# Sreyan88/audio-ssl

Measured on AMD Instinct MI355X. Metric: upstream clips/sec (1s@16kHz, 64-mel), higher is better.
Workload: dtype bf16; 1 GPU; delores-m upstream step (log-mel + 2 views + q/k conv encoders + MoCo + 3 Barlow heads + bwd + SGD), 1 s @ 16 kHz, 64 mel, batch 512/GPU, queue 65536; global_batch=512, parallelism=dp1

## Files before the change

audio-ssl_amd/src/engine.py:

```python
import os

import torch

from src import _native as N

import os as _os
_STEM_VALU = _os.environ.get("AUDIOSSL_STEM_VALU") == "1"
BN_MOMENTUM = 0.1
BN_EPS = 1e-5
_BN_FUSED = _os.environ.get("AUDIOSSL_BN_FUSED", "1") != "0"


ONE_STREAM = os.environ.get("AUDIOSSL_ONE_STREAM", "0") == "1"


_CAPTURE_ORIGIN = []


class capture_scope:

    def __enter__(self):
        _CAPTURE_ORIGIN.append(torch.cuda.current_stream())
        return self

# ... 91 lines not shown
    n = src.numel()
    if src.dtype == torch.float32 and dst.dtype == torch.float32 and src.is_contiguous() and dst.is_contiguous() and n % 1024 == 0 \
            and n // 1024 < (1 << 31) and src.data_ptr() % 16 == 0 and dst.data_ptr() % 16 == 0:
        N.call("tile_rows", src, dst, n // 1024, n // 1024, 1, 1.0, 1024)
    else:
        dst.copy_(src)
    return dst


def _ksplit(M, Nn, K, target=512):
    tiles = ((M + 127) // 128) * ((Nn + 127) // 128)
    return int(max(1, min(target // max(tiles, 1), (K // 64) // 32)))


def gemm(dtype, ta, tb, M, Nn, K, A, lda, B, ldb, C, ldc, alpha=1.0, bias=None, relu=0, keep=None, ldk=0, keep_scale=1.0,
         gate=None, ldg=0, out_f32=0, atomic=0, ksplit=1, resid=None, ldr=0):
    N.call("gemm", dtype, ta, tb, M, Nn, K, float(alpha), A, lda, B, ldb, C, ldc, bias, relu, keep, ldk, float(keep_scale),
           gate, ldg, out_f32, atomic, ksplit, resid, ldr)


def linear_fwd(dtype, X, W, M, Nout, K, bias=None, relu=0, keep=None, keep_scale=1.0, out=None, out_f32=0):
    if out is None and dtype == N.BF16 and out_f32 and not relu and keep is None and M * Nout <= (1 << 16) and K >= 1024 and K % 512 == 0:
        out = ARENA.zeros((M, Nout), torch.float32, like=X)
        gemm(dtype, 0, 0, M, Nout, K, X, K, W, K, out, Nout, bias=bias, out_f32=1, atomic=1, ksplit=min(8, K // 256))
        return out
    if out is None:
        out = _empty((M, Nout), torch.float32 if (out_f32 or dtype == 0) else torch.bfloat16, like=X)
    gemm(dtype, 0, 0, M, Nout, K, X, K, W, K, out, Nout, bias=bias, relu=relu, keep=keep, ldk=Nout, keep_scale=keep_scale,
         out_f32=out_f32)
    return out


def linear_bwd_w(dtype, dY, X, dW, M, Nout, K, dw_zero=False):
    ks = _ksplit(Nout, K, M)
    atomic = 1 if (ks > 1 or dtype != N.BF16) else (0 if dw_zero else 2)
    gemm(dtype, 1, 1, Nout, K, M, dY, Nout, X, K, dW, K, out_f32=1, atomic=atomic, ksplit=ks)


def linear_bwd_x(dtype, dY, W, M, Nout, K, alpha=1.0, gate=None, out=None, out_f32=0):
    if out is None:
        out = _empty((M, K), torch.float32 if (out_f32 or dtype == N.F32) else torch.bfloat16, like=dY)
    gemm(dtype, 0, 1, M, K, Nout, dY, Nout, W, K, out, K, alpha=alpha, gate=gate, ldg=K, out_f32=out_f32)
    return out


GD = N.F32

HP = False


def set_high_precision(flag):
    global HP
    HP = bool(flag)


SYNC_BN = None


class SyncBN:
    def __init__(self, group=None):
        import torch.distributed as dist
        self.dist, self.group = dist, group
        self.world = dist.get_world_size(group)

    def all_reduce(self, t):
        self.dist.all_reduce(t, group=self.group)
        return t


def set_sync_bn(sync):
    global SYNC_BN
    SYNC_BN = sync if (sync is not None and sync.world > 1) else None


def _ad(dtype):
    return N.F32 if (HP or dtype == N.F32) else dtype


def pooled_dtype(dtype):
    return torch.float32


def center_cast(Y, groups, B):
    C = Y.shape[1]
    yc = _empty((groups * B, C), torch.bfloat16, like=Y)
    cmean = _empty((groups, C), torch.float32, like=Y)
    N.call("center_cast", Y, yc, cmean, groups, B, C)
    return yc, cmean


def colsum_add(dtype, X, M, C, dst, tmp=None):
    tmp = tmp if tmp is not None else ARENA.scratch((C,), torch.float64, X)
    N.call("colstats", dtype, X, 1, M, C, C, 0, tmp, None)
    N.call("add_d2f", tmp, dst, C)


def cast(dtype, src, n=None):
    if dtype == N.F32:
        return src
    out = torch.empty(src.shape, dtype=torch.bfloat16, device=src.device)
    N.call("cast", dtype, src, out, src.numel())
    return out


class EncoderCtx:
    pass


def _bn_train(dtype, Y, M, C, gamma, beta, rm, rv, update_running, groups=1):
    sq = ARENA.scratch((2, groups * C), torch.float64, Y)
    N.call("colstats", dtype, Y, groups, M, C, C, 1, sq[0], sq[1])
    if SYNC_BN is not None:
        SYNC_BN.all_reduce(sq)
        M = M * SYNC_BN.world
    st = _empty((4, groups * C), torch.float32, like=Y)
    N.call("bn_finalize", sq[0], sq[1], groups, float(M), C, gamma, beta, rm if update_running else None,
           rv if update_running else None, BN_MOMENTUM, BN_EPS, st[0], st[1], st[2], st[3])
    return st[0], st[1], st[2], st[3]


def bn_train_apply(dtype, ad, a, M, C, gamma, beta, rm, rv, update_running, groups, relu, out):
    if M <= 1024 and C % 32 == 0 and _BN_FUSED and SYNC_BN is None:
        st = _empty((4, groups * C), torch.float32, like=a)
        N.call("colbn_train_fwd", dtype, ad, a, gamma, beta, rm if update_running else None, rv if update_running else None,
               BN_MOMENTUM, BN_EPS, relu, groups, M, C, out, st[0], st[1], st[2], st[3])
        return st[0], st[1], st[2], st[3]
    st = _bn_train(ad, a, M, C, gamma, beta, rm, rv, update_running, groups)
    N.call("colbn_fwd", dtype, ad, a, st[0], st[1], relu, out, groups, M, C)
    return st


def _bn_eval(like, C, gamma, beta, rm, rv):
    scale, shift = _empty((C,), torch.float32, like=like), _empty((C,), torch.float32, like=like)
    N.call("bn_eval_affine", gamma, beta, rm, rv, BN_EPS, C, scale, shift)
    return scale, shift


_WGRAD_WS = {}


def _wgrad_workspace(device):
    key = device.index if device.index is not None else torch.cuda.current_device()
    ws = _WGRAD_WS.get(key)
    if ws is None:
        ws = _WGRAD_WS[key] = torch.empty(256 * 64 * 576, dtype=torch.float32, device=device)
    return ws


STAT_REPLICAS = 8
LOSS_REPLICAS = 32
_BN_STATS_P = os.environ.get("AUDIOSSL_BN_STATS_P", "1") != "0"
_DP1_BF16 = os.environ.get("AUDIOSSL_DP1_BF16", "1") != "0"
_CONV_POOL = os.environ.get("AUDIOSSL_CONV_POOL", "1") != "0"
_CONV_WS = int(os.environ.get("AUDIOSSL_CONV_WS", "1")) != 0


def _conv_block_fwd(dtype, Pin, Nimg, Ti, Fi, W, bias, bn, train, update_running, col, packed=None, keep_y=True):
    td = N.torch_dtype(dtype)
    if packed is not None:
        Wf, Wd = packed
    else:
        Wf, Wd = _empty((64, 576), td, like=Pin), _empty((64, 576), td, like=Pin)
        N.call("pack_conv_w", dtype, W, Wf, Wd)
    M = Nimg * Ti * Fi
    ad = _ad(dtype)
    gamma, beta, rm, rv = bn
    fused = dtype == N.BF16 and Fi in (16, 32)
    if fused and ad == dtype and _CONV_POOL and _CONV_WS and Ti % 2 == 0 and M * 128 < 0x7FFFFF00:
        rep = STAT_REPLICAS if (train and SYNC_BN is None) else 1
        sq = ARENA.scratch((rep, 2, 64), torch.float64, Pin)
        Y = _empty((M, 64), td, like=Pin) if keep_y else None
        Pout = _empty((Nimg, Ti // 2, Fi // 2, 64), td, like=Pin)
        N.call("conv3x3_pool_fwd", Pin, Wf, bias, gamma, Y, Pout, sq[0, 0], sq[0, 1], rep, Nimg, Ti, Fi)
        if train and SYNC_BN is None:
            st = _empty((4, 64), torch.float32, like=Pin)
            N.call("bn_relu_pooled_train_fwd", dtype, Pout, sq[0, 0], sq[0, 1], rep, float(M), gamma, beta, rm if update_running else None,
                   rv if update_running else None, BN_MOMENTUM, BN_EPS, Pout, st[0], st[1], st[2], st[3], Nimg, Ti // 2, Fi // 2)
            return Y, Pout, (st[0], st[1], st[2], st[3]), Wf, Wd
        if train:
            st = _empty((4, 64), torch.float32, like=Pin)
            sq = sq[0]
            SYNC_BN.all_reduce(sq)
            N.call("bn_finalize", sq[0], sq[1], 1, float(M * SYNC_BN.world), 64, gamma, beta, rm if update_running else None,
                   rv if update_running else None, BN_MOMENTUM, BN_EPS, st[0], st[1], st[2], st[3])
            scale, shift, mean, rstd = st[0], st[1], st[2], st[3]
        else:
            scale, shift = _bn_eval(Pin, 64, gamma, beta, rm, rv)
            mean = rstd = None
        N.call("bn_relu_pooled_fwd", dtype, Pout, scale, shift, Pout, Nimg, Ti // 2, Fi // 2)
        return Y, Pout, (scale, shift, mean, rstd), Wf, Wd
    Y = _empty((M, 64), N.torch_dtype(ad), like=Pin)
    rep = STAT_REPLICAS if (fused and train and SYNC_BN is None) else 1
    sq = ARENA.scratch((rep, 2, 64), torch.float64, Pin) if (fused and train) else None
    if fused:
        N.call("conv3x3_fwd", Pin, Wf, bias, Y, int(ad == N.F32), None if sq is None else sq[0, 0], None if sq is None else sq[0, 1],
               rep, Nimg, Ti, Fi)
    else:
        N.call("im2col3x3", dtype, Pin, col, Nimg, Ti, Fi)
        gemm(dtype, 0, 0, M, 64, 576, col, 576, Wf, 576, Y, 64, bias=bias, out_f32=int(ad == N.F32))
    Pout = _empty((Nimg, Ti // 2, Fi // 2, 64), td, like=Pin)
    if train and fused and SYNC_BN is None:
        st = _empty((4, 64), torch.float32, like=Pin)
        N.call("bn_relu_pool_train_fwd", dtype, ad, Y, sq[0, 0], sq[0, 1], rep, float(M), gamma, beta, rm if update_running else None,
               rv if update_running else None, BN_MOMENTUM, BN_EPS, Pout, st[0], st[1], st[2], st[3], Nimg, Ti, Fi)
        return Y, Pout, (st[0], st[1], st[2], st[3]), Wf, Wd
    if train and fused:
        st = _empty((4, 64), torch.float32, like=Pin)
        sq = sq[0]
        SYNC_BN.all_reduce(sq)
        N.call("bn_finalize", sq[0], sq[1], 1, float(M * SYNC_BN.world), 64, gamma, beta, rm if update_running else None,
               rv if update_running else None, BN_MOMENTUM, BN_EPS, st[0], st[1], st[2], st[3])
        scale, shift, mean, rstd = st[0], st[1], st[2], st[3]
    elif train:
        scale, shift, mean, rstd = _bn_train(ad, Y, M, 64, gamma, beta, rm, rv, update_running)
    else:
        scale, shift = _bn_eval(Y, 64, gamma, beta, rm, rv)
        mean = rstd = None
    N.call("bn_relu_pool_fwd", dtype, ad, Y, scale, shift, Pout, Nimg, Ti, Fi)
    return Y, Pout, (scale, shift, mean, rstd), Wf, Wd


def _col_buffer(dtype, Nimg, T1, F1, like):
    if dtype == N.BF16 and F1 in (16, 32):
        return None
    return _empty((Nimg * T1 * F1, 576), N.torch_dtype(dtype), like=like)


MOM_SLOT = 17 * 54


def stem_fused(dtype, train=True):
    return bool(train) and dtype == N.BF16 and not HP and not _STEM_VALU and SYNC_BN is None


def stem_moments_pair(xa, xb=None):
    Nimg, _, F, T = xa.shape
    assert xb is None or xb.shape == xa.shape
    mom = ARENA.scratch((1 if xb is None else 2, MOM_SLOT), torch.float64, xa)
    N.call("conv1_moments_pair", xa.reshape(Nimg, F, T).contiguous(), None if xb is None else xb.reshape(Nimg, F, T).contiguous(),
           Nimg, F, T, mom)
    return mom


def encoder_forward(P, x, dtype, keep=None, p_drop=0.3, train=True, update_running=True, want_layers=True, Wc=None,
                    layer_out=None, before_fc=None, stem_moments=None, need_bwd=True, lens=None, hop=160):
    Nimg, _, F, T = x.shape
    assert F == 64, "the HIP encoder is built for n_mels = 64 (the reference's only setting)"
    td = N.torch_dtype(dtype)
    c = EncoderCtx()
    c.P = P
    c.dtype, c.N, c.F, c.T, c.train, c.p_drop = dtype, Nimg, F, T, train, p_drop
    c.need_bwd = need_bwd
    ragged = lens is not None
    if ragged:
        assert not train and not need_bwd, "a ragged batch runs in eval mode without a backward (BatchNorm on running statistics)"
        assert T % 8 == 0, "a ragged batch is padded to a multiple of 8 frames"
        assert lens.dtype == torch.int32 and lens.is_cuda and tuple(lens.shape) == (Nimg,), "lens: int32 [N] on the device"
    img = x.reshape(Nimg, F, T).contiguous()
    c.img = img
    w1 = P["features_1.0.weight"].reshape(64, 9)
    b1 = P["features_1.0.bias"]
    g1, be1 = P["features_1.1.weight"], P["features_1.1.bias"]
    c.stem_mfma = dtype == N.BF16 and not HP and not _STEM_VALU
    fused = stem_fused(dtype, train)
    assert stem_moments is None or fused, "precomputed stem moments are for the fused bf16 training stem only"
    rm1 = rv1 = None
    if train:
        c.sc1, c.sh1, c.mean1, c.rstd1 = (_empty((64,), torch.float32, like=x) for _ in range(4))
        rm1 = P["features_1.1.running_mean"] if update_running else None
        rv1 = P["features_1.1.running_var"] if update_running else None
    if fused:
        c.mom1 = stem_moments if stem_moments is not None else stem_moments_pair(x)[0]
    elif train:
        c.mom1 = ARENA.scratch((16 * 54,), torch.float64, x)
        if SYNC_BN is None:
            N.call("conv1_stats", img, Nimg, F, T, w1, b1, g1, be1, rm1, rv1, BN_MOMENTUM, BN_EPS, c.mom1, c.sc1, c.sh1, c.mean1, c.rstd1)
        else:
            N.call("conv1_moments", img, Nimg, F, T, c.mom1)
            mom_g = SYNC_BN.all_reduce(c.mom1[:54].clone())
            N.call("conv1_finalize", mom_g, w1, b1, g1, be1, rm1, rv1, BN_MOMENTUM, BN_EPS, float(Nimg * F * T * SYNC_BN.world),
                   c.sc1, c.sh1, c.mean1, c.rstd1)
    else:
        c.sc1, c.sh1 = _bn_eval(x, 64, g1, be1, P["features_1.1.running_mean"], P["features_1.1.running_var"])
    T1, F1 = T // 2, F // 2
    c.P1 = _empty((Nimg, T1, F1, 64), td, like=x)
    x1 = x2 = x3 = None
    if want_layers:
        x1, x2, x3 = layer_out if layer_out is not None else (_empty((Nimg, f * 64), torch.float32 if ragged else td, like=x)
                                                              for f in (F // 2, F // 4, F // 8))
    x1_fused = c.stem_mfma and x1 is not None and x1.dtype == torch.float32 and x1.is_contiguous() and not ragged
    x1_parts = _empty((4, Nimg, (F // 2) * 64), torch.float32, like=x) if x1_fused else None
    if fused:
        N.call("conv1_fwd_train", img, Nimg, F, T, c.mom1, float(Nimg * F * T), w1, b1, g1, be1, rm1, rv1, BN_MOMENTUM, BN_EPS,
               c.sc1, c.sh1, c.mean1, c.rstd1, c.P1, x1_parts)
    else:
        N.call("conv1_fwd", dtype if (dtype == N.F32 or c.stem_mfma) else 2, img, Nimg, F, T, w1, b1, c.sc1, c.sh1, c.P1, x1_parts)
    if ragged:
        N.call("tail_mask", dtype, c.P1, lens, hop, 1, Nimg, T1, F1 * 64)
    col = _col_buffer(dtype, Nimg, T1, F1, x)
    bn2 = (P["features_2.1.weight"], P["features_2.1.bias"], P["features_2.1.running_mean"], P["features_2.1.running_var"])
    packs = [_empty((64, 576), td, like=x) for _ in range(4)]
    N.call("pack_conv_w2", dtype, P["features_2.0.weight"], packs[0], packs[1], P["features_3.0.weight"], packs[2], packs[3])
    c.Y2, c.P2, c.st2, c.W2f, c.W2d = _conv_block_fwd(dtype, c.P1, Nimg, T1, F1, P["features_2.0.weight"],
                                                       P["features_2.0.bias"], bn2, train, update_running, col, packed=packs[:2],
                                                       keep_y=need_bwd)
    T2, F2 = T1 // 2, F1 // 2
# ... 311 lines not shown
    vp = ctypes.c_void_p
    arrs = (_harr(ctypes.c_int, Ns), _harr(ctypes.c_int, Ks), _harr(vp, As), _harr(ctypes.c_long, ldas), _harr(vp, Bs),
            _harr(ctypes.c_long, ldbs), _harr(vp, Ps), _harr(vp, Moms), _harr(vp, Shadows if Shadows is not None else [None] * n),
            _harr(ctypes.c_long, ldps))
    if N.PROFILE is not None:
        N.PROFILE_NOTE = (float(sum(2.0 * M * nn * kk for nn, kk in zip(Ns, Ks))),
                          float(sum(2.0 * kk * (M + nn) + M * nn * (16.0 + (2.0 if Shadows is not None else 0.0)) for nn, kk in zip(Ns, Ks))))
    lr, mu, wd, gs, gs_dev = hyper
    N.call("gemm_multi_sgd", n, ta, tb, M, adr(arrs[0]), adr(arrs[1]), float(alpha), adr(arrs[2]), adr(arrs[3]), adr(arrs[4]), adr(arrs[5]),
           adr(arrs[6]), adr(arrs[7]), adr(arrs[8]), adr(arrs[9]), float(lr), float(mu), float(wd), float(gs), gs_dev)


def _heads_wgrad_split(D, kmax, M, nh):
    return _ksplit(D, kmax, M, max(256 // nh, 1))


def heads_wgrads_store(D, kins, M, grads_zero=True):
    nh = len(kins)
    return bool(grads_zero) and all(_heads_wgrad_split(D, k, M, nh) == 1 for k in (D, max(kins)))


def barlow_heads_forward_backward(PPs, Gs, Ys, dtype, lambds, scale_losses, loss_outs, update_running=True, backward=True,
                                  Wcs=None, grads_zero=False, dy_ready=None, sgd=None):
    import ctypes
    nh = len(Ys)
    B = Ys[0].shape[0] // 2
    M = 2 * B
    td = N.torch_dtype(dtype)
    dev = Ys[0].device
    W = Wcs if Wcs is not None else [tuple(cast(dtype, PP[f"projector.{i}.weight"]) for i in (0, 3, 6)) for PP in PPs]
    D = W[0][0].shape[0]
    kins = [Y.shape[1] for Y in Ys]
    ad = _ad(dtype)
    if dtype != N.BF16 or ad != N.BF16 or B > 1024 or D % 32:
        raise RuntimeError("grouped Barlow heads: bf16 path with B <= 1024 only")
    H = range(nh)
    vp, fl, adr = ctypes.c_void_p, ctypes.c_float, ctypes.addressof
    new = lambda rows, cols, t: [torch.empty(rows, cols, dtype=t, device=dev) for _ in H]

    def layer(xs, ws, ks, prefix, affine, relu):
        a = new(M, D, td)
        gemm_multi(0, 0, M, D, ks, xs, ks, ws, ks, a, D)
        out, st = new(M, D, td), new(4, 2 * D, torch.float32)
        par = lambda suffix, on=True: _harr(vp, [PP[prefix + suffix] if on else None for PP in PPs])
        arrs = (_harr(vp, a), par(".weight", affine), par(".bias", affine), par(".running_mean", update_running),
                par(".running_var", update_running), _harr(vp, out), _harr(vp, st))
        _multi_check(a, out, st)
        N.call("colbn_train_fwd_multi", nh, ad, adr(arrs[0]), adr(arrs[1]), adr(arrs[2]), adr(arrs[3]), adr(arrs[4]),
               BN_MOMENTUM, BN_EPS, relu, 2, B, D, adr(arrs[5]), adr(arrs[6]))
        return a, st, out
    ycs = [torch.empty(M, k, dtype=torch.bfloat16, device=dev) for k in kins]
    cms = [torch.empty(2, k, dtype=torch.float32, device=dev) for k in kins]
    _multi_check(list(Ys), ycs, cms)
    if any(Y.dtype != torch.float32 or k % 32 for Y, k in zip(Ys, kins)):
        raise RuntimeError("grouped Barlow heads: fp32 inputs with width % 32 == 0")
    arrs = (_harr(vp, list(Ys)), _harr(vp, ycs), _harr(vp, cms), _harr(ctypes.c_int, kins))
    N.call("center_cast_multi", nh, adr(arrs[0]), adr(arrs[1]), adr(arrs[2]), adr(arrs[3]), 2, B)
    a1, st1, h1 = layer(ycs, [W[h][0] for h in H], kins, "projector.1", True, 1)

    def shift_running():
        rms = [PP["projector.1.running_mean"] for PP in PPs]
        w0 = [W[h][0] for h in H]
        _multi_check(w0, rms)
        arrs = (_harr(vp, w0), _harr(vp, cms), _harr(vp, rms), _harr(ctypes.c_int, kins))
        N.call("shift_running_mean_multi", nh, adr(arrs[0]), adr(arrs[1]), adr(arrs[2]), D, adr(arrs[3]), 2, BN_MOMENTUM)
    shift_late = update_running and backward and dy_ready is not None
    if update_running and not shift_late:
        shift_running()
    a2, st2, h2 = layer(h1, [W[h][1] for h in H], [D] * nh, "projector.4", True, 1)
    z, st0, zn = layer(h2, [W[h][2] for h in H], [D] * nh, "bn", False, 0)
    dc = new(D, D, td)
    coefs = [(lambds[h] if lambds[h] else 1.0) * scale_losses[h] for h in H]
    dsc = [2.0 * c / B for c in coefs]
    if all(l.numel() == LOSS_REPLICAS for l in loss_outs) and D % 64 == 0:
        _multi_check([zn[h] for h in H], dc, list(loss_outs))
        arrs = (_harr(ctypes.c_int, [B] * nh), _harr(vp, [zn[h][:B] for h in H]), _harr(ctypes.c_long, [D] * nh),
                _harr(vp, [zn[h][B:] for h in H]), _harr(ctypes.c_long, [D] * nh), _harr(vp, dc), _harr(fl, coefs), _harr(fl, dsc),
                _harr(vp, list(loss_outs)))
        if N.PROFILE is not None:
            N.PROFILE_NOTE = float(nh * 2.0 * D * D * B)
        N.call("gemm_multi_barlow", nh, D, adr(arrs[0]), 1.0 / B, adr(arrs[1]), adr(arrs[2]), adr(arrs[3]), adr(arrs[4]), adr(arrs[5]),
               adr(arrs[6]), adr(arrs[7]), adr(arrs[8]))
    else:
        cm = new(D, D, torch.float32)
        gemm_multi(1, 1, D, D, [B] * nh, [zn[h][:B] for h in H], [D] * nh, [zn[h][B:] for h in H], [D] * nh, cm, D,
                   alpha=1.0 / B, out_f32=1)
        arrs = (_harr(vp, cm), _harr(fl, coefs), _harr(fl, dsc), _harr(vp, dc), _harr(vp, list(loss_outs)))
        _multi_check(list(loss_outs))
        N.call("barlow_loss_multi", nh, adr(arrs[0]), D, adr(arrs[1]), adr(arrs[2]), adr(arrs[3]), adr(arrs[4]))
    if not backward:
        return [None] * nh
    dzn = new(M, D, torch.float32)
    gemm_multi(0, 0, B, D, [D] * nh, [zn[h][B:] for h in H], [D] * nh, dc, [D] * nh, [dzn[h][:B] for h in H], D, out_f32=1)
    gemm_multi(0, 1, B, D, [D] * nh, [zn[h][:B] for h in H], [D] * nh, dc, [D] * nh, [dzn[h][B:] for h in H], D, out_f32=1)

    def bn_bwd(a, dh, st, relu, names):
        out = new(M, D, td)
        grads = lambda k: _harr(vp, [Gs[h][names[k]] if names else None for h in H])
        arrs = (_harr(vp, a), _harr(vp, dh), _harr(vp, st), _harr(vp, out), grads(0), grads(1))
        _multi_check(a, dh, st)
        N.call("colbn_bwd_multi", nh, ad, GD, adr(arrs[0]), adr(arrs[1]), adr(arrs[2]), relu, 2, B, D, adr(arrs[3]),
               adr(arrs[4]), adr(arrs[5]))
        return out

    def wgrad(dys, xs, name, ks):
        split = _heads_wgrad_split(D, max(ks), M, nh)
        if sgd is not None:
            if split != 1 or Wcs is None:
                raise RuntimeError("fused SGD needs unsplit weight gradients and the flat weight shadows")
            li = {"projector.0.weight": 0, "projector.3.weight": 1, "projector.6.weight": 2}[name]
            gemm_multi_sgd(1, 1, D, ks, [M] * nh, dys, [D] * nh, xs, ks, [PPs[h][name] for h in H], [sgd["momentum"][h][name] for h in H],
                           [W[h][li] for h in H], ks, sgd["hyper"])
            return
        gemm_multi(1, 1, D, ks, [M] * nh, dys, [D] * nh, xs, ks, [Gs[h][name] for h in H], ks, out_f32=1,
                   atomic=1 if split > 1 else (0 if grads_zero else 2), ksplit=split)

    def dgrad(dys, ws, Ks, rows):
        out = [torch.empty(rows, k, dtype=torch.float32, device=dev) for k in Ks]
        gemm_multi(0, 1, rows, Ks, [D] * nh, [dy[:rows] for dy in dys], [D] * nh, ws, Ks, out, Ks, out_f32=1)
        return out
    later = []
    defer = (lambda fn: later.append(fn)) if dy_ready is not None else (lambda fn: fn())
    dz = bn_bwd(z, dzn, st0, 0, None)
    defer(lambda: wgrad(dz, h2, "projector.6.weight", [D] * nh))
    dh2 = dgrad(dz, [W[h][2] for h in H], [D] * nh, M)
    da2 = bn_bwd(a2, dh2, st2, 1, ("projector.4.weight", "projector.4.bias"))
    defer(lambda: wgrad(da2, h1, "projector.3.weight", [D] * nh))
    dh1 = dgrad(da2, [W[h][1] for h in H], [D] * nh, M)
    da1 = bn_bwd(a1, dh1, st1, 1, ("projector.1.weight", "projector.1.bias"))
    defer(lambda: wgrad(da1, ycs, "projector.0.weight", kins))
    dy = dgrad(da1, [W[h][0] for h in H], kins, B)
    if dy_ready is not None:
        dy_ready()
    if shift_late:
        shift_running()
    for fn in later:
        fn()
    return dy


def moco_forward_backward(dtype, q, k, queue, queue_shadow, temperature, loss_out, backward=True):
    B, dim = q.shape
    K = queue.shape[1]
    td = N.torch_dtype(dtype)
    qn, kn = _empty((B, dim), td, like=q), _empty((B, dim), td, like=q)
    qn32, kn32 = _empty((B, dim), torch.float32, like=q), _empty((B, dim), torch.float32, like=q)
    qinv, kinv = _empty((B,), torch.float32, like=q), _empty((B,), torch.float32, like=q)
    lpos = _empty((B,), torch.float32, like=q)
    N.call("moco_prep", dtype, q, k, B, dim, 1.0 / temperature, qn, qn32, qinv, kn, kn32, kinv, lpos)
    lse = _empty((B,), torch.float32, like=q)
    dlpos = _empty((B,), torch.float32, like=q)
    Pm = None
    if dtype == N.BF16 and K % 8 == 0 and dim % 8 == 0:
        nslot = (K + 63) // 64
        part = _empty((B, nslot, 2), torch.float32, like=q)
        N.call("moco_logits", 1, qn, queue_shadow, B, K, dim, 1.0 / temperature, part, None, 0.0, None)
        N.call("moco_lse_merge", lpos, part, B, nslot, 1.0 / (B * temperature), lse, loss_out, dlpos)
        if not backward:
            return None, kn32
        Pm = _empty((B, K), td, like=q)
        N.call("moco_logits", 2, qn, queue_shadow, B, K, dim, 1.0 / temperature, None, lse, 1.0 / (B * temperature), Pm)
    else:
        lneg = _empty((B, K), torch.float32, like=q)
        gemm(dtype, 0, 1, B, K, dim, qn, dim, queue_shadow, K, lneg, K, alpha=1.0 / temperature, out_f32=1)
        N.call("moco_ce_fwd", lpos, lneg, B, K, lse, loss_out)
        if not backward:
            return None, kn32
        Pm = _empty((B, K), td, like=q)
        N.call("moco_ce_bwd", dtype, lpos, lneg, lse, B, K, 1.0 / (B * temperature), Pm, dlpos)
    dqn = ARENA.zeros((B, dim), torch.float32, device=q.device)
    gemm(dtype, 0, 0, B, dim, K, Pm, K, queue_shadow, K, dqn, dim, out_f32=1, atomic=1, ksplit=_ksplit(B, dim, K, 256))
    dq = _empty((B, dim), td, like=q)
    N.call("l2norm_bwd", dtype, dqn, dlpos, kn32, qn32, qinv, B, dim, dq)
    return dq, kn32
```

include/audiossl_hip.h:

```cpp
#ifndef AUDIOSSL_HIP_H
#define AUDIOSSL_HIP_H

#include <stdint.h>

#ifdef __cplusplus
extern "C" {
#endif

#define AUDIOSSL_OK 0
#define AUDIOSSL_EINVAL (-1)
#define AUDIOSSL_ELAUNCH (-2)
#define AUDIOSSL_EALIGN (-3)

int audiossl_logmel_fwd(const float* wave, float* out, int B, int L, int T, int n_fft, int hop, int n_mels, int taps,
                        const float* win, const float* tw, const float* melw, const int* mel_start, float eps_pow,
                        float eps_log, int apply_log, void* stream);
int audiossl_logmel_ragged_fwd(const float* wave, const int* lens, const int* lens_host, float* out, int B, int Lmax, int Tmax,
                               int n_fft, int hop, int n_mels, int taps, const float* win, const float* tw, const float* melw,
                               const int* mel_start, float eps_pow, float eps_log, int apply_log, void* stream);

int audiossl_fbank_fwd(const float* wave, const int* lens, const int* partner, const float* lam, float* clip_mean,
                       const int* bands, const int* bands_host, float* out, int B, int Lmax, int win_len, int shift, int n_fft, int n_mels,
                       int taps, int T_target, const float* win, const float* tw, const float* melw, const int* mel_start,
                       float preemph, float eps_log, float mean, float std, int skip_norm, int time_major, void* stream);
// ... 15 lines not shown
                           const int* off_r, const double* eta_l, const double* eta_r, const double* win, const double* delta,
                           int nwin, int index_step, void* stream);

int audiossl_pcm_window(const void* pcm, long pcm_bytes, const long long* tab, const long long* tab_host, float* out, int B,
                        int unit, int align, void* stream);

int audiossl_kmix_cluster(const float* views, const float* centroids, int n_views, int F, int T, int K, int* cluster,
                          void* stream);
int audiossl_kmix_apply(const float* views, const float* ring, const int* slot, const float* coef, int n_views, int n,
                        int log_mix, float* out, void* stream);
int audiossl_mask_fill(float* x, const int* tab, int n_img, int max_masks, int F, int T, int zero_fill, void* stream);

int audiossl_conv1_stats(const float* img, int N, int F, int T, const float* w, const float* bias, const float* gamma,
                         const float* beta, float* running_mean, float* running_var, float momentum, float eps,
                         double* mom, float* scale, float* shift, float* save_mean, float* save_rstd, void* stream);
#define AUDIOSSL_CONV1_XL_PARTS 4
int audiossl_conv1_fwd(int dtype, const float* img, int N, int F, int T, const float* w, const float* bias,
                       const float* scale, const float* shift, void* out, float* xl, void* stream);
#define AUDIOSSL_CONV1_MOM_SLOT (17 * 54)
int audiossl_conv1_moments_pair(const float* img_a, const float* img_b, int N, int F, int T, double* mom, void* stream);
int audiossl_conv1_fwd_train(const float* img, int N, int F, int T, double* mom, double count, const float* w, const float* bias,
                             const float* gamma, const float* beta, float* running_mean, float* running_var, float momentum,
                             float eps, float* scale, float* shift, float* save_mean, float* save_rstd, void* out, float* xl,
                             void* stream);
int audiossl_conv1_bwd(int dtype, int conv_dtype, const float* img, int N, int F, int T, const float* w, const float* bias,
                       const float* gamma, const float* scale, const float* shift, const float* mean, const float* rstd,
                       const double* mom, const void* dP, const void* dxl, float* acc, float* dW, float* dbias,
                       float* dgamma, float* dbeta, void* stream);

int audiossl_colstats(int dtype, const void* x, int groups, long M, int C, long ld, int want_sq, double* sum,
                      double* sumsq, void* stream);
int audiossl_bn_finalize(const double* sum, const double* sumsq, int groups, double count, int C, const float* gamma,
                         const float* beta, float* running_mean, float* running_var, float momentum, float eps,
                         float* scale, float* shift, float* save_mean, float* save_rstd, void* stream);
int audiossl_bn_relu_pool_fwd(int dtype, int ydtype, const void* Y, const float* scale, const float* shift, void* P, int N,
                              int Ti, int Fi, void* stream);
int audiossl_bn_relu_pool_train_fwd(int dtype, int ydtype, const void* Y, const double* sum, const double* sumsq, int stat_replicas,
                                    double count, const float* gamma, const float* beta, float* running_mean, float* running_var,
                                    float momentum, float eps, void* P, float* scale, float* shift, float* save_mean, float* save_rstd,
                                    int N, int Ti, int Fi, void* stream);
int audiossl_bn_relu_pooled_fwd(int dtype, const void* Praw, const float* scale, const float* shift, void* P, int N, int To, int Fo,
                                void* stream);
int audiossl_bn_relu_pooled_train_fwd(int dtype, const void* Praw, const double* sum, const double* sumsq, int stat_replicas,
                                      double count, const float* gamma, const float* beta, float* running_mean, float* running_var,
                                      float momentum, float eps, void* P, float* scale, float* shift, float* save_mean,
                                      float* save_rstd, int N, int To, int Fo, void* stream);
int audiossl_tmean_fwd(int dtype, int out_f32, const void* P, void* xl, int N, int To, int Fo, void* stream);
int audiossl_tmean3_fwd(int dtype, int out_f32, const void* P1, void* x1, const float* x1_parts, int To1, int Fo1, const void* P2,
                        void* x2, int To2, int Fo2, const void* P3, void* x3, int To3, int Fo3, int N, void* stream);
int audiossl_bn_relu_pool_bwd(int dtype, int ydtype, int gdtype, const void* Y, const void* dP, const void* dxl, const float* scale,
                              const float* shift, const float* mean, const float* rstd, float* stat, void* dY,
                              float* dgamma, float* dbeta, int N, int Ti, int Fi, void* stream);
int audiossl_bn_relu_pool_bwd_p(int dtype, int ydtype, int gdtype, const void* Y, const void* P, const void* dP, const void* dxl,
                                const float* scale, const float* shift, const float* mean, const float* rstd, float* stat, void* dY,
                                float* dgamma, float* dbeta, int N, int Ti, int Fi, void* stream);
int audiossl_conv1_moments(const float* img, int N, int F, int T, double* mom, void* stream);
int audiossl_conv1_finalize(double* mom_totals, const float* w, const float* bias, const float* gamma, const float* beta,
                            float* running_mean, float* running_var, float momentum, float eps, double count, float* scale,
                            float* shift, float* save_mean, float* save_rstd, void* stream);
int audiossl_conv1_bwd_sums(int dtype, int conv_dtype, const float* img, int N, int F, int T, const float* w, const float* bias,
                            const float* gamma, const float* scale, const float* shift, const float* mean, const float* rstd,
                            const double* mom, const void* dP, const void* dxl, float* acc, float* lstat, void* stream);
int audiossl_conv1_bwd_finalize(const float* acc, const double* mom, const float* w, const float* bias, const float* gamma,
                                const float* mean, const float* rstd, double count_global, const float* gstat, float* dW,
                                float* dbias, float* dgamma, float* dbeta, void* stream);
int audiossl_bn_relu_pool_bwd_stats(int dtype, int ydtype, int gdtype, const void* Y, const void* dP, const void* dxl,
                                    const float* scale, const float* shift, const float* mean, const float* rstd, float* stat,
                                    int N, int Ti, int Fi, void* stream);
int audiossl_bn_relu_pool_bwd_apply(int dtype, int ydtype, int gdtype, const void* Y, const void* dP, const void* dxl,
                                    const float* scale, const float* shift, const float* mean, const float* rstd, float* stat,
                                    const float* gstat, double count_global, void* dY, float* dgamma, float* dbeta, int N, int Ti,
                                    int Fi, void* stream);
int audiossl_colbn_bwd_stats(int dtype, int adtype, int gdtype, const void* a, const void* dh, const float* scale,
                             const float* shift, const float* mean, const float* rstd, int relu, int groups, long M, int C,
                             double* tmp, void* stream);
int audiossl_colbn_bwd_apply(int dtype, int adtype, int gdtype, const void* a, const void* dh, const float* scale,
                             const float* shift, const float* mean, const float* rstd, int relu, int groups, long M, int C,
                             const double* sums, double count, void* da, void* stream);
int audiossl_im2col3x3(int dtype, const void* X, void* col, int N, int Ti, int Fi, void* stream);
int audiossl_pack_conv_w(int dtype, const float* W, void* Wf, void* Wd, void* stream);
int audiossl_pack_conv_w2(int dtype, const float* Wa, void* Wfa, void* Wda, const float* Wb, void* Wfb, void* Wdb, void* stream);
int audiossl_unpack_conv_dw(const float* dWp, float* dW, void* stream);

int audiossl_conv3x3_fwd(const void* X, const void* W, const float* bias, void* Y, int out_f32, double* sum,
                         double* sumsq, int stat_replicas, int N, int Ti, int Fi, void* stream);
int audiossl_conv3x3_pool_fwd(const void* X, const void* W, const float* bias, const float* gamma, void* Y, void* Praw, double* sum,
                              double* sumsq, int stat_replicas, int N, int Ti, int Fi, void* stream);
int audiossl_conv3x3_wgrad(const void* dY, const void* X, float* dWp, float* workspace, long workspace_floats, int N, int Ti,
                           int Fi, void* stream);

int audiossl_gemm(int dtype, int trans_a, int trans_b, int M, int N, int K, float alpha, const void* A, long lda,
                  const void* B, long ldb, void* C, long ldc, const float* bias, int relu, const uint8_t* keep, long ldk,
                  float keep_scale, const void* gate, long ldg, int out_f32, int atomic, int ksplit, const float* resid,
                  long ldr, void* stream);

int audiossl_gemm_dropout(int trans_a, int trans_b, int M, int N, int K, float alpha, const void* A, long lda, const void* B,
                          long ldb, void* C, long ldc, const float* bias, int relu, unsigned long long seed, float p,
                          const long long* counter, float keep_scale, void* stream);

int audiossl_gemm_multi(int count, int trans_a, int trans_b, int M, const int* N, const int* K, float alpha,
                        const void* const* A, const long* lda, const void* const* B, const long* ldb, void* const* C,
                        const long* ldc, int out_f32, int atomic, int ksplit, void* stream);
int audiossl_gemm_multi_sgd(int count, int trans_a, int trans_b, int M, const int* Nv, const int* K, float alpha,
                            const void* const* A, const long* lda, const void* const* B, const long* ldb, float* const* P,
                            float* const* Mom, void* const* Shadow, const long* ldp, float lr, float momentum, float weight_decay,
                            float grad_scale, const float* grad_scale_dev, void* stream);
int audiossl_gemm_multi_barlow(int count, int D, const int* K, float alpha, const void* const* A, const long* lda,
                               const void* const* B, const long* ldb, void* const* dc, const float* coef, const float* dscale,
                               float* const* loss_rep, void* stream);

int audiossl_maxmean_fwd(int dtype, int out_f32, const void* H, void* y, uint8_t* arg, int N, int Tt, int D, void* stream);
int audiossl_maxmean_bwd(int dtype, int gdtype, const void* dy, const uint8_t* arg, const void* H, void* dA, int N, int Tt,
                         int D, void* stream);

int audiossl_tail_mask(int dtype, void* P, const int* lens, int hop, int shift, int N, int To, long row_elems, void* stream);
int audiossl_tmean3_ragged_fwd(int dtype, const void* P1, float* x1, int To1, int Fo1, const void* P2, float* x2, int To2, int Fo2,
                               const void* P3, float* x3, int To3, int Fo3, const int* lens, int hop, int N, void* stream);
int audiossl_meanmax_ragged_fwd(int dtype, const void* H, float* mean, float* maxmean, const int* lens, int hop, int shift, int N,
                                int Tt, int D, void* stream);

int audiossl_colbn_fwd(int dtype, int adtype, const void* a, const float* scale, const float* shift, int relu, void* h,
                       int groups, long M, int C, void* stream);
int audiossl_colbn_train_fwd(int dtype, int adtype, const void* a, const float* gamma, const float* beta,
                             float* running_mean, float* running_var, float momentum, float eps, int relu, int groups,
                             long M, int C, void* h, float* scale, float* shift, float* save_mean, float* save_rstd,
                             void* stream);
int audiossl_colbn_bwd(int dtype, int adtype, int gdtype, const void* a, const void* dh, const float* scale, const float* shift, const float* mean,
                       const float* rstd, int relu, int groups, long M, int C, double* tmp, void* da, float* dgamma,
                       float* dbeta, void* stream);
int audiossl_colbn_train_fwd_multi(int count, int adtype, const void* const* a, const float* const* gamma,
                                   const float* const* beta, float* const* running_mean, float* const* running_var,
                                   float momentum, float eps, int relu, int groups, long M, int C, void* const* h,
                                   float* const* stats, void* stream);
int audiossl_colbn_bwd_multi(int count, int adtype, int gdtype, const void* const* a, const void* const* dh,
                             const float* const* stats, int relu, int groups, long M, int C, void* const* da,
                             float* const* dgamma, float* const* dbeta, void* stream);
int audiossl_barlow_loss_multi(int count, const float* const* c, int D, const float* coef, const float* dscale,
                               void* const* dc, float* const* loss_out, void* stream);
int audiossl_add_d2f(const double* src, float* dst, int n, void* stream);
int audiossl_barlow_loss(int dtype, const float* c, int D, float coef, float dscale, void* dc, float* loss_out,
                         void* stream);

int audiossl_l2norm_fwd(int dtype, const float* q, int B, int D, void* qn, float* qn32, float* inv_norm, void* stream);
int audiossl_moco_prep(int dtype, const float* q, const float* k, int B, int D, float scale, void* qn, float* qn32, float* qinv,
                       void* kn, float* kn32, float* kinv, float* lpos, void* stream);
int audiossl_rowdot(const float* a, const float* b, int B, int D, float scale, float* out, void* stream);
int audiossl_moco_ce_fwd(const float* lpos, const float* lneg, int B, int K, float* lse, float* loss_out, void* stream);
int audiossl_moco_ce_bwd(int dtype, const float* lpos, const float* lneg, const float* lse, int B, int K, float gscale,
                         void* P, float* dlpos, void* stream);
int audiossl_moco_logits(int mode, const void* qn, const void* queue, int B, int K, int dim, float inv_t, float* part,
                         const float* lse, float gscale, void* P, void* stream);
int audiossl_moco_lse_merge(const float* lpos, const float* part, int B, int nslot, float gscale, float* lse,
                            float* loss_out, float* dlpos, void* stream);
int audiossl_l2norm_bwd(int dtype, const float* dqn, const float* dlpos, const float* kn32, const float* qn32,
                        const float* inv_norm, int B, int D, void* dq, void* stream);
int audiossl_enqueue(int dtype, const float* keys, int B, int D, int K, int ptr, long long* ptr_dev, float* queue, void* shadow,
                     void* stream);
int audiossl_ema_update(float* pk, const float* pq, long n, float m, void* shadow, void* stream);

int audiossl_set_prezeroed(int on);
int audiossl_last_kernel(char* name, int capacity);

int audiossl_sgd_momentum(float* p, float* g, float* buf, long n, float lr, float momentum, float weight_decay,
                          int first, float grad_scale, const float* grad_scale_dev, void* shadow_bf16, int zero_grad,
                          void* stream);
int audiossl_sgd_momentum_segments(float* p, float* g, float* buf, const long* segs, int nseg, long max_n, float lr, float momentum,
                                   float weight_decay, int first, float grad_scale, const float* grad_scale_dev, void* shadow_bf16,
                                   int zero_grad, void* stream);
int audiossl_zero_segments(float* g, const long* segs, int nseg, long max_n, void* stream);
int audiossl_cast(int dtype, const float* src, void* dst, long n, void* stream);
int audiossl_cast_back(int dtype, const void* src, float* dst, long n, void* stream);
int audiossl_dropout_mask(uint8_t* keep, long n, unsigned long long seed, float p, const long long* counter, void* stream);
int audiossl_relu_bwd(int dtype, const void* g, const void* h, void* out, long n, void* stream);
int audiossl_bn_eval_affine(const float* gamma, const float* beta, const float* running_mean, const float* running_var,
                            float eps, int C, float* scale, float* shift, void* stream);
int audiossl_axpy(float* y, const float* x, float a, long n, void* stream);
int audiossl_split_bf16(const float* x, void* hi, void* lo, long n, void* stream);
int audiossl_center_cast(const float* y, void* yc, float* cmean, int groups, long M, int C, void* stream);
int audiossl_shift_running_mean(const void* W, const float* cmean, float* running_mean, int D, int K, int groups,
                                float momentum, void* stream);
int audiossl_center_cast_multi(int count, const float* const* y, void* const* yc, float* const* cmean, const int* C, int groups,
                               long M, void* stream);
int audiossl_shift_running_mean_multi(int count, const void* const* W, const float* const* cmean, float* const* running_mean,
                                      int D, const int* K, int groups, float momentum, void* stream);

int audiossl_ntxent_fwd(const float* sim, int N, int B, float* lse, float* loss_out, void* stream);
int audiossl_ntxent_bwd(int dtype, const float* sim, const float* lse, int N, int B, float gscale, void* dsim, void* stream);

int audiossl_row_argmax(const float* dot, long N, int K, long long* assign, void* stream);
int audiossl_kmeans_accumulate(const float* x, const long long* assign, long N, int K, int D, float* sums, int* counts,
                               void* stream);
int audiossl_kmeans_update(const float* sums, const int* counts, int K, int D, float* centroids, void* stream);
int audiossl_kmeans_update_mean(const float* sums, const int* counts, int K, int D, float* centroids, void* stream);
int audiossl_row_sqnorm(const float* x, int rows, int D, float scale, float* out, void* stream);
int audiossl_ce_rows(int dtype, const float* logits, const long long* target, int B, int K, int ignore_index, int* cnt,
                     float* loss_out, void* dlogits, void* stream);

int audiossl_unfused_loss(int gdtype, const float* z1, const float* z2, const float* z3, const float* t,
                          const long long* label, int B, int C, long ld, float alpha, float beta, float gamma,
                          float* loss4, void* dz1, void* dz2, void* dz3, void* dt, void* stream);

int audiossl_knn_workspace(int Nq, long Nb, int k, long* bytes);
int audiossl_knn_topk(const void* q, const void* bank, int Nq, long Nb, int D, int k, float* top_sim, int* top_idx,
                      void* workspace, long workspace_bytes, void* stream);
int audiossl_knn_vote(const float* top_sim, const int* top_idx, const long long* bank_label, int Nq, int k, long Nb,
                      float inv_t, long long* pred, float* conf, void* stream);

int audiossl_cka_workspace(int n, int p, int q, long* bytes);
int audiossl_cka_center(const float* x, int n, int p, float* out, void* stream);
int audiossl_cka_sigma2(const float* x, int n, int p, double* sigma2, long long* count, void* workspace,
                        long workspace_bytes, void* stream);
int audiossl_cka_hsic(const float* x, const float* y, int n, int p, int q, int kernel, double sigma,
                      const double* sigma2_x, const double* sigma2_y, double* out, double* rowsum_k,
                      double* rowsum_l, void* workspace, long workspace_bytes, void* stream);

int audiossl_knn_graph_workspace(int n, int k, long* bytes);
int audiossl_knn_graph_l2(const float* x, int n, int d, int k, int* idx, float* d2, void* workspace, long workspace_bytes,
                          void* stream);
int audiossl_pic_workspace(int n, int k, long* bytes);
int audiossl_pic_build(const int* idx, const float* d2, int n, int k, double sigma, int* rowptr, int* col, double* w, int* nnz,
                       void* workspace, long workspace_bytes, void* stream);
int audiossl_pic_power(const int* rowptr, const int* col, const double* w, int n, long cap, double alpha, int iters, double* v,
                       void* workspace, long workspace_bytes, void* stream);
int audiossl_pic_assign(const int* rowptr, const int* col, const double* w, const double* v, int n, long cap, int* label,
                        int* count, void* workspace, long workspace_bytes, void* stream);

int audiossl_silhouette_workspace(int n, long* bytes);
int audiossl_silhouette(const float* xs, int n, int d, const int* seg, const int* seg_host, int K, double* s, void* workspace,
                        long workspace_bytes, void* stream);

int audiossl_tsne_workspace(int n, int k, long* bytes);
int audiossl_tsne_calibrate(const float* d2, int n, int k, double perplexity, float* p_cond, float* beta, void* stream);
int audiossl_tsne_symmetrize(const int* idx, const float* p_cond, int n, int k, int* rowptr, int* col, float* p, int* nnz,
                             void* workspace, long workspace_bytes, void* stream);
int audiossl_tsne_repulsion(const float* y, int n, float* rep, double* Z, void* workspace, long workspace_bytes, void* stream);
int audiossl_tsne_gradient(const int* rowptr, const int* col, const float* p, long cap, const float* y, const float* rep,
                           const double* Z, int n, double exaggeration, float* grad, double* kl, void* workspace,
                           long workspace_bytes, void* stream);
int audiossl_tsne_update(const float* grad, int n, double momentum, double learning_rate, float* y, float* update, float* gains,
                         void* stream);

int audiossl_bce_rows(int dtype, const float* logits, const float* targets, long N, int C, float* loss_out, void* dlogits,
                      void* stream);
int audiossl_tagging_workspace(long N, int C, long* bytes);
int audiossl_tagging_stats(const float* scores, const unsigned char* targets, long N, int C, int* npos, long long* auc_num2,
                           double* ap, double* auc, void* workspace, long workspace_bytes, void* stream);

int audiossl_softmax_rows_fwd(const float* x, float* y, int M, int C, void* stream);
int audiossl_softmax_rows_bwd(const float* y, const float* gy, float* gx, int M, int C, void* stream);

int audiossl_attn_fwd(const void* qkv, void* out, float* lse, int B, int S, int H, float scale, void* stream);
int audiossl_attn_bwd(const void* qkv, const void* out, const void* dout, const float* lse, void* dqkv, int B, int S, int H,
                      float scale, void* stream);
int audiossl_layernorm_fwd(const float* x, const float* gamma, const float* beta, void* y, float* y32, float* mean, float* rstd,
                           int M, int C, float eps, void* stream);
int audiossl_layernorm_bwd(const float* dy, const float* x, const float* mean, const float* rstd, const float* gamma,
                           float* dres, float* dgamma, float* dbeta, int M, int C, void* stream);
int audiossl_gelu_fwd(const void* a, void* h, long n, void* stream);
int audiossl_gelu_bwd(const void* a, const void* dh, void* da, long n, void* stream);
int audiossl_patch_unfold(const float* x, void* out, int B, int F, int T, int fstride, int tstride, void* stream);
int audiossl_tile_rows(const float* src, float* out, long rows, int period, int group, float scale, int C, void* stream);
int audiossl_adamw(float* p, const float* g, float* m, float* v, long n, float lr, float beta1, float beta2, float eps,
                   float weight_decay, float grad_scale, const long long* step, void* stream);

int audiossl_mvit_pool_fwd(const void* qkv, int ldq, int col0, const float* w, const float* gamma, const float* beta, float* out,
                           float* z, float* mean, float* rstd, int B, int heads, int d, int H, int W, int Ho, int Wo, int sh, int sw,
                           float eps, void* stream);
int audiossl_mvit_pool_bwd(const void* qkv, int ldq, int col0, const float* w, const float* gamma, const float* dout, const float* z,
                           const float* mean, const float* rstd, float* dz, float* dw, float* dgamma, float* dbeta, void* dqkv, int B,
                           int heads, int d, int H, int W, int Ho, int Wo, int sh, int sw, void* stream);
int audiossl_mvit_attn_fwd(const float* q, const float* k, const float* v, const float* rh, const float* rw, const int* ih,
                           const int* iw, void* out, float* lse, int B, int heads, int d, int qh, int qw, int kh, int kw, int nrh,
                           int nrw, int residual, float scale, void* stream);
int audiossl_mvit_attn_bwd(const float* q, const float* k, const float* v, const float* rh, const float* rw, const int* ih,
                           const int* iw, const void* dout, const float* lse, float* dq, float* dk, float* dv, float* drh, float* drw,
                           int B, int heads, int d, int qh, int qw, int kh, int kw, int nrh, int nrw, int residual, float scale,
                           void* stream);
int audiossl_tokpool_max_fwd(const float* x, float* y, void* arg, int B, int H, int W, int C, int kh, int kw, int sh, int sw,
                             void* stream);
int audiossl_tokpool_max_bwd(const float* dy, const void* arg, float* dx, int B, int H, int W, int C, int kh, int kw, int sh, int sw,
                             void* stream);

int audiossl_lars_step(float* p, const float* g, float* mu, const void* seg, int n_seg, const float* lr, float weight_decay,
                       float momentum, float eta, float grad_scale, double* norms, void* stream);
int audiossl_larc_step(float* p, const float* g, float* mu, const void* seg, int n_seg, float lr, float weight_decay,
                       float momentum, float trust_coefficient, float eps, int clip, float grad_scale, double* norms,
                       void* stream);

#ifdef __cplusplus
}
#endif
#endif
```

Before: 273,400 clips/s.

## Add specialised MoCo logits pass and dq kernels with queue-stationary MFMA tiles

```diff
diff --git a/audio-ssl_amd/csrc/moco.hip b/audio-ssl_amd/csrc/moco.hip
--- /dev/null
+++ b/audio-ssl_amd/csrc/moco.hip
@@ -0,0 +1,231 @@
+#include "common.h"
+
+namespace {
+
+constexpr int DIM = 128;
+constexpr int PASS_SLAB = 256;
+constexpr float LOG2E = 1.44269504088896340736f;
+constexpr int STAGE_PITCH = 72;
+
+__device__ __forceinline__ void wave_lds_sync() {
+    __builtin_amdgcn_fence(__ATOMIC_RELEASE, "wavefront");
+    __builtin_amdgcn_wave_barrier();
+    __builtin_amdgcn_fence(__ATOMIC_ACQUIRE, "wavefront");
+}
+
+__device__ __forceinline__ void load_qn_tile(bf16x8 (&f)[8], const bf16* __restrict__ qn, int row, int h) {
+    const bf16* p = qn + (long)row * DIM + 8 * h;
+#pragma unroll
+    for (int ks = 0; ks < 8; ++ks) f[ks] = *reinterpret_cast<const bf16x8*>(p + ks * 16);
+}
+
+template <int MODE>
+__global__ __launch_bounds__(256) void moco_pass_kernel(const bf16* __restrict__ qn, const bf16* __restrict__ queue, int B, int K,
+                                                        float inv_t, float* __restrict__ part, const float* __restrict__ lse,
+                                                        float gscale, bf16* __restrict__ P) {
+    __shared__ __attribute__((aligned(16))) bf16 stage[MODE == 2 ? 4 * 32 * STAGE_PITCH : 8];
+    const int lane = threadIdx.x & 63, wave = threadIdx.x >> 6;
+    const int l31 = lane & 31, h = lane >> 5;
+    const int ntile = B >> 5, nslot = K >> 6;
+    const float c2 = inv_t * LOG2E;
+    for (int slab = blockIdx.x; slab * PASS_SLAB < K; slab += gridDim.x) {
+        const int col0 = slab * PASS_SLAB + wave * 64;
+        bf16x8 a[2][8];
+#pragma unroll
+        for (int blk = 0; blk < 2; ++blk) {
+            const bf16* qc = queue + col0 + 32 * ((l31 >> 2) & 1) + 16 * blk + (l31 & 3) + 4 * (l31 >> 3);
+#pragma unroll
+            for (int ks = 0; ks < 8; ++ks)
+#pragma unroll
+                for (int u = 0; u < 8; ++u) a[blk][ks][u] = qc[(long)(ks * 16 + 8 * h + u) * K];
+        }
+        bf16x8 cur[8], nxt[8];
+        load_qn_tile(cur, qn, l31, h);
+        for (int t = 0; t < ntile; ++t) {
+            const int row = t * 32 + l31;
+            if (t + 1 < ntile) load_qn_tile(nxt, qn, row + 32, h);
+            f32x16 acc0 = {0}, acc1 = {0};
+#pragma unroll
+            for (int ks = 0; ks < 8; ++ks) {
+                acc0 = __builtin_amdgcn_mfma_f32_32x32x16_bf16(a[0][ks], cur[ks], acc0, 0, 0, 0);
+                acc1 = __builtin_amdgcn_mfma_f32_32x32x16_bf16(a[1][ks], cur[ks], acc1, 0, 0, 0);
+            }
+            if constexpr (MODE == 1) {
+                float m = acc0[0];
+#pragma unroll
+                for (int r = 0; r < 16; ++r) { m = fmaxf(m, acc0[r]); m = fmaxf(m, acc1[r]); }
+                const float mc = m * c2;
+                float s = 0.f;
+#pragma unroll
+                for (int r = 0; r < 16; ++r)
+                    s += __builtin_amdgcn_exp2f(__builtin_fmaf(acc0[r], c2, -mc)) + __builtin_amdgcn_exp2f(__builtin_fmaf(acc1[r], c2, -mc));
+                const float m2 = __shfl_xor(m, 32, 64), s2 = __shfl_xor(s, 32, 64);
+                const float mm = fmaxf(m, m2);
+                s = s * __builtin_amdgcn_exp2f((m - mm) * c2) + s2 * __builtin_amdgcn_exp2f((m2 - mm) * c2);
+                const float mm_out = mm * inv_t;
+                if (h == 0) *reinterpret_cast<float2*>(part + ((long)row * nslot + (col0 >> 6)) * 2) = make_float2(mm_out, s);
+            } else {
+                const float lc = lse[row] * LOG2E;
+                bf16* st = stage + wave * 32 * STAGE_PITCH;
+                bf16x8 o[4];
+#pragma unroll
+                for (int r = 0; r < 16; ++r) {
+                    o[r >> 3][r & 7] = (bf16)(__builtin_amdgcn_exp2f(__builtin_fmaf(acc0[r], c2, -lc)) * gscale);
+                    o[2 + (r >> 3)][r & 7] = (bf16)(__builtin_amdgcn_exp2f(__builtin_fmaf(acc1[r], c2, -lc)) * gscale);
+                }
+#pragma unroll
+                for (int c = 0; c < 4; ++c) *reinterpret_cast<bf16x8*>(st + l31 * STAGE_PITCH + 32 * h + 8 * c) = o[c];
+                wave_lds_sync();
+                bf16* dst = P + (long)(t * 32 + (lane >> 3)) * K + col0 + 8 * (lane & 7);
+#pragma unroll
+                for (int it = 0; it < 4; ++it) {
+                    const bf16x8 v = *reinterpret_cast<const bf16x8*>(st + (it * 8 + (lane >> 3)) * STAGE_PITCH + 8 * (lane & 7));
+                    *reinterpret_cast<bf16x8*>(dst + (long)it * 8 * K) = v;
+                }
+                wave_lds_sync();
+            }
+#pragma unroll
+            for (int ks = 0; ks < 8; ++ks) cur[ks] = nxt[ks];
+        }
+    }
+}
+
+constexpr int DQ_ROWS = 128;
+constexpr size_t DQ_LDS = 2 * sizeof(float) * DQ_ROWS * DIM;
+
+template <bool FULL>
+__device__ __forceinline__ void dq_load(bf16x8 (&a)[8], bf16x8 (&b)[8], const bf16* __restrict__ pa, const bf16* __restrict__ pb,
+                                        long K, int k, int nbi) {
+#pragma unroll
+    for (int i = 0; i < 8; ++i)
+        if (FULL || i < nbi) a[i] = *reinterpret_cast<const bf16x8*>(pa + (long)i * 16 * K + k);
+#pragma unroll
+    for (int j = 0; j < 8; ++j) b[j] = *reinterpret_cast<const bf16x8*>(pb + (long)j * 16 * K + k);
+}
+
+template <bool FULL>
+__device__ __forceinline__ void dq_mma(f32x4 (&acc)[8][8], const bf16x8 (&a)[8], const bf16x8 (&b)[8], int nbi) {
+#pragma unroll
+    for (int i = 0; i < 8; ++i)
+        if (FULL || i < nbi) {
+#pragma unroll
+            for (int j = 0; j < 8; ++j) acc[i][j] = __builtin_amdgcn_mfma_f32_16x16x32_bf16(a[i], b[j], acc[i][j], 0, 0, 0);
+        }
+}
+
+template <bool FULL, int I0>
+__device__ __forceinline__ void dq_fold_half(const f32x4 (&acc)[8][8], float* __restrict__ red, float* __restrict__ out, int wave,
+                                             int lane, int nbi) {
+    constexpr int TILE = 4 * 8 * 64 * 4;
+    float* mine = red + wave * TILE;
+#pragma unroll
+    for (int i = I0; i < I0 + 4; ++i)
+        if (FULL || i < nbi) {
+#pragma unroll
+            for (int j = 0; j < 8; ++j) *reinterpret_cast<f32x4*>(mine + (((i - I0) * 8 + j) * 64 + lane) * 4) = acc[i][j];
+        }
+    __syncthreads();
+#pragma unroll 2
+    for (int q = 0; q < 8; ++q) {
+        const int blk = wave + 4 * q, i = I0 + (blk >> 3), j = blk & 7;
+        if (FULL || i < nbi) {
+            const float* src = red + (blk * 64 + lane) * 4;
+            f32x4 v = *reinterpret_cast<const f32x4*>(src);
+#pragma unroll
+            for (int w = 1; w < 4; ++w) v += *reinterpret_cast<const f32x4*>(src + w * TILE);
+#pragma unroll
+            for (int r = 0; r < 4; ++r) unsafeAtomicAdd(out + (i * 16 + r) * DIM + j * 16, v[r]);
+        }
+    }
+    __syncthreads();
+}
+
+template <bool FULL>
+__global__ __launch_bounds__(256) void moco_dq_kernel(const bf16* __restrict__ P, const bf16* __restrict__ queue, int B, int K,
+                                                      int L, int rowtiles, int nslab, float* __restrict__ dqn) {
+    extern __shared__ __attribute__((aligned(16))) float red[];
+    const int lane = threadIdx.x & 63, wave = threadIdx.x >> 6;
+    const int l15 = lane & 15, g = lane >> 4;
+    int rt, slab;
+    if ((nslab & 7) == 0) { rt = (blockIdx.x >> 3) % rowtiles; slab = (blockIdx.x & 7) + 8 * (blockIdx.x / (8 * rowtiles)); }
+    else { rt = blockIdx.x % rowtiles; slab = blockIdx.x / rowtiles; }
+    const int row0 = rt * DQ_ROWS;
+    const int nbi = FULL ? 8 : min(8, (B - row0) >> 4);
+    const int k0 = slab * L, k1 = min(K, k0 + L);
+
+    f32x4 acc[8][8];
+#pragma unroll
+    for (int i = 0; i < 8; ++i)
+#pragma unroll
+        for (int j = 0; j < 8; ++j) acc[i][j] = f32x4{0.f, 0.f, 0.f, 0.f};
+    const bf16* pa = P + (long)(row0 + l15) * K + 8 * g;
+    const bf16* pb = queue + (long)l15 * K + 8 * g;
+    const int kw = k0 + 64 * wave;
+    const int nstage = (k1 - k0) >> 7;
+    const auto kof = [kw](int s) { return kw + 256 * (s >> 1) + 32 * (s & 1); };
+    bf16x8 a0[8], b0[8], a1[8], b1[8], a2[8], b2[8];
+    dq_load<FULL>(a0, b0, pa, pb, K, kof(0), nbi);
+    dq_load<FULL>(a1, b1, pa, pb, K, kof(1), nbi);
+    for (int s = 0; s < nstage; s += 3) {
+        if (s + 2 < nstage) dq_load<FULL>(a2, b2, pa, pb, K, kof(s + 2), nbi);
+        dq_mma<FULL>(acc, a0, b0, nbi);
+        if (s + 1 < nstage) {
+            if (s + 3 < nstage) dq_load<FULL>(a0, b0, pa, pb, K, kof(s + 3), nbi);
+            dq_mma<FULL>(acc, a1, b1, nbi);
+        }
+        if (s + 2 < nstage) {
+            if (s + 4 < nstage) dq_load<FULL>(a1, b1, pa, pb, K, kof(s + 4), nbi);
+            dq_mma<FULL>(acc, a2, b2, nbi);
+        }
+    }
+    float* out = dqn + (long)(row0 + 4 * g) * DIM + l15;
+    dq_fold_half<FULL, 0>(acc, red, out, wave, lane, nbi);
+    dq_fold_half<FULL, 4>(acc, red, out, wave, lane, nbi);
+}
+
+int moco_shape_ok(int B, int K, int dim) {
+    return B > 0 && K > 0 && dim == DIM && B % 32 == 0 && K % PASS_SLAB == 0;
+}
+
+}
+
+extern "C" int audiossl_moco_pass(int mode, const void* qn, const void* queue, int B, int K, int dim, float inv_t, float* part,
+                                  const float* lse, float gscale, void* P, void* stream) {
+    ASSL_REQUIRE(qn && queue && (mode == 1 || mode == 2));
+    ASSL_REQUIRE(mode == 1 ? part != nullptr : (lse != nullptr && P != nullptr));
+    ASSL_REQUIRE(moco_shape_ok(B, K, dim) && inv_t > 0.f);
+    if (!ASSL_ALIGNED16(qn) || !ASSL_ALIGNED16(queue)) return ASSL_EALIGN;
+    if (mode == 1 ? (((uintptr_t)part) & 7) != 0 : !ASSL_ALIGNED16(P)) return ASSL_EALIGN;
+    const dim3 grid((unsigned)min(K / PASS_SLAB, 256));
+    const bf16* q = static_cast<const bf16*>(qn);
+    const bf16* qu = static_cast<const bf16*>(queue);
+    if (mode == 1)
+        hipLaunchKernelGGL(moco_pass_kernel<1>, grid, dim3(256), 0, S_(stream), q, qu, B, K, inv_t, part, lse, gscale,
+                           static_cast<bf16*>(nullptr));
+    else
+        hipLaunchKernelGGL(moco_pass_kernel<2>, grid, dim3(256), 0, S_(stream), q, qu, B, K, inv_t, part, lse, gscale,
+                           static_cast<bf16*>(P));
+    ASSL_LAUNCH_CHECK();
+}
+
+extern "C" int audiossl_moco_dq(const void* P, const void* queue, int B, int K, int dim, float* dqn, void* stream) {
+    ASSL_REQUIRE(P && queue && dqn);
+    ASSL_REQUIRE(moco_shape_ok(B, K, dim));
+    if (!ASSL_ALIGNED16(P) || !ASSL_ALIGNED16(queue) || (((uintptr_t)dqn) & 3) != 0) return ASSL_EALIGN;
+    const int rowtiles = ceil_div(B, DQ_ROWS);
+    const int want = 256 / rowtiles > 0 ? 256 / rowtiles : 1;
+    const int L = ceil_div(ceil_div(K, want), 256) * 256;
+    const int nslab = ceil_div(K, L);
+    const dim3 grid((unsigned)(rowtiles * nslab));
+    const bf16* p = static_cast<const bf16*>(P);
+    const bf16* qu = static_cast<const bf16*>(queue);
+    static const bool lds_ok =
+        hipFuncSetAttribute(reinterpret_cast<const void*>(moco_dq_kernel<true>), hipFuncAttributeMaxDynamicSharedMemorySize, (int)DQ_LDS) == hipSuccess &&
+        hipFuncSetAttribute(reinterpret_cast<const void*>(moco_dq_kernel<false>), hipFuncAttributeMaxDynamicSharedMemorySize, (int)DQ_LDS) == hipSuccess;
+    if (!lds_ok) return ASSL_ELAUNCH;
+    if (B % DQ_ROWS == 0)
+        hipLaunchKernelGGL(moco_dq_kernel<true>, grid, dim3(256), DQ_LDS, S_(stream), p, qu, B, K, L, rowtiles, nslab, dqn);
+    else
+        hipLaunchKernelGGL(moco_dq_kernel<false>, grid, dim3(256), DQ_LDS, S_(stream), p, qu, B, K, L, rowtiles, nslab, dqn);
+    ASSL_LAUNCH_CHECK();
+}
diff --git a/audio-ssl_amd/src/engine.py b/audio-ssl_amd/src/engine.py
--- a/audio-ssl_amd/src/engine.py
+++ b/audio-ssl_amd/src/engine.py
@@ -267,6 +267,7 @@
 _BN_STATS_P = os.environ.get("AUDIOSSL_BN_STATS_P", "1") != "0"
 _DP1_BF16 = os.environ.get("AUDIOSSL_DP1_BF16", "1") != "0"
 _CONV_POOL = os.environ.get("AUDIOSSL_CONV_POOL", "1") != "0"
+_MOCO_QS = os.environ.get("AUDIOSSL_MOCO_QS", "1") != "0"
 _CONV_WS = int(os.environ.get("AUDIOSSL_CONV_WS", "1")) != 0
 
 
@@ -884,14 +885,22 @@
     dlpos = _empty((B,), torch.float32, like=q)
     Pm = None
     if dtype == N.BF16 and K % 8 == 0 and dim % 8 == 0:
+        qs = _MOCO_QS and dim == 128 and B % 32 == 0 and K % 256 == 0
+        logits = "moco_pass" if qs else "moco_logits"
         nslot = (K + 63) // 64
         part = _empty((B, nslot, 2), torch.float32, like=q)
-        N.call("moco_logits", 1, qn, queue_shadow, B, K, dim, 1.0 / temperature, part, None, 0.0, None)
+        N.call(logits, 1, qn, queue_shadow, B, K, dim, 1.0 / temperature, part, None, 0.0, None)
         N.call("moco_lse_merge", lpos, part, B, nslot, 1.0 / (B * temperature), lse, loss_out, dlpos)
         if not backward:
             return None, kn32
         Pm = _empty((B, K), td, like=q)
-        N.call("moco_logits", 2, qn, queue_shadow, B, K, dim, 1.0 / temperature, None, lse, 1.0 / (B * temperature), Pm)
+        N.call(logits, 2, qn, queue_shadow, B, K, dim, 1.0 / temperature, None, lse, 1.0 / (B * temperature), Pm)
+        if qs:
+            dqn = ARENA.zeros((B, dim), torch.float32, device=q.device)
+            N.call("moco_dq", Pm, queue_shadow, B, K, dim, dqn)
+            dq = _empty((B, dim), td, like=q)
+            N.call("l2norm_bwd", dtype, dqn, dlpos, kn32, qn32, qinv, B, dim, dq)
+            return dq, kn32
     else:
         lneg = _empty((B, K), torch.float32, like=q)
         gemm(dtype, 0, 1, B, K, dim, qn, dim, queue_shadow, K, lneg, K, alpha=1.0 / temperature, out_f32=1)
diff --git a/include/audiossl_hip.h b/include/audiossl_hip.h
--- a/include/audiossl_hip.h
+++ b/include/audiossl_hip.h
@@ -191,6 +191,9 @@
                          const float* lse, float gscale, void* P, void* stream);
 int audiossl_moco_lse_merge(const float* lpos, const float* part, int B, int nslot, float gscale, float* lse,
                             float* loss_out, float* dlpos, void* stream);
+int audiossl_moco_pass(int mode, const void* qn, const void* queue, int B, int K, int dim, float inv_t, float* part,
+                       const float* lse, float gscale, void* P, void* stream);
+int audiossl_moco_dq(const void* P, const void* queue, int B, int K, int dim, float* dqn, void* stream);
 int audiossl_l2norm_bwd(int dtype, const float* dqn, const float* dlpos, const float* kn32, const float* qn32,
                         const float* inv_norm, int B, int D, void* dq, void* stream);
 int audiossl_enqueue(int dtype, const float* keys, int B, int D, int K, int ptr, long long* ptr_dev, float* queue, void* shadow,
```

Result: no change. 273,100 clips/s (-0.1%).
